# tgialoimtr/cnn_lstm_ctc_ocr

Hardware: AMD Instinct MI355X
Metric: line-crops/sec (train step) at 32x256 bs=256; CER vs ref (higher is better)
Workload: dtype bf16

## Files before the change

### cnn_lstm_ctc_ocr_amd/csrc/gemm.hip

```cpp
#include <atomic>
#include <cstdlib>
#include <type_traits>

#include "gemm.h"
#include "mfma_util.h"

namespace ocrk {

template <int AM, typename CT>
__device__ __forceinline__ const CT* a_addr(const GemmParams& p, const CT* A, int m, int k, bool& ok) {
    if constexpr (AM == A_ROWK) {
        ok = m < p.M && k < p.K;
        return A + (int64_t)m * p.lda + k;
    } else if constexpr (AM == A_COLK) {
        ok = m < p.M && k < p.K;
        return A + (int64_t)k * p.lda + m;
    } else {
        int pix, kidx;
        if constexpr (AM == A_IM2COL_T) { pix = k; kidx = m; ok = k < p.K && m < p.M; }
        else { pix = m; kidx = k; ok = m < p.M && k < p.K; }
        const int C = p.convC, W = p.convW, H = p.convH;
        int tap = kidx / C, c = kidx - tap * C;
        int kh = tap / 3, kw = tap - kh * 3;
        int w = pix % W, t2 = pix / W, h = t2 % H, b = t2 / H;
        int hh, ww;
        if constexpr (AM == A_IM2COL_FLIP) { hh = h - kh + 1; ww = w - kw + 1; }
        else { hh = h + kh - 1; ww = w + kw - 1; }
        ok = ok && hh >= 0 && hh < H && ww >= 0 && ww < W;
        return A + (((int64_t)b * H + hh) * W + ww) * C + c;
    }
}

template <int BMD, typename CT>
__device__ __forceinline__ const CT* b_addr(const GemmParams& p, const CT* B, int n, int k, bool& ok) {
    ok = n < p.N && k < p.K;
    if constexpr (BMD == B_NK) return B + (int64_t)n * p.ldb + k;
    else return B + (int64_t)k * p.ldb + n;
}

template <typename CT, int AM, int BMD, int TBM, int TBN, bool X3 = false>
__global__ void __launch_bounds__(256) gemm_kernel(const GemmParams p) {
    static_assert(!X3 || sizeof(CT) == 4, "bf16x3 splits fp32 operands");
    using RT = typename std::conditional<X3, unsigned short, typename RawT<CT>::T>::type;
    constexpr int BK = 32, LDK = BK + 8;
    constexpr int WM = TBM / 2, WN = TBN / 2, TM = WM / 16, TN = WN / 16;
    constexpr bool A_K = (AM == A_ROWK || AM == A_IM2COL || AM == A_IM2COL_FLIP);
    constexpr bool B_K = (BMD == B_NK);
    constexpr bool BF = sizeof(CT) == 2;
    constexpr bool A_TR = BF && !A_K, B_TR = BF && !B_K;
    constexpr bool PERM = A_TR || B_TR;
    constexpr int LDA_R = TBM + 16, LDB_R = TBN + 16;
    constexpr int A_ELEMS = A_TR ? BK * LDA_R : TBM * LDK;
    constexpr int B_ELEMS = B_TR ? BK * LDB_R : TBN * LDK;
    constexpr int NVA = (TBM * BK / 8 + 255) / 256;
    constexpr int NVB = (TBN * BK / 8 + 255) / 256;
    __shared__ __attribute__((aligned(16))) RT sA[2][X3 ? 2 * A_ELEMS : A_ELEMS];
    __shared__ __attribute__((aligned(16))) RT sB[2][X3 ? 2 * B_ELEMS : B_ELEMS];

    const int tid = threadIdx.x, lane = tid & 63, wave = tid >> 6;
    const int wm = wave >> 1, wn = wave & 1;
    const int m0 = blockIdx.x * TBM, n0 = blockIdx.y * TBN;
    const int zb = blockIdx.z / p.splits, zs = blockIdx.z - zb * p.splits;
    const CT* A = reinterpret_cast<const CT*>(p.A) + zb * p.strideA;
    const CT* B = reinterpret_cast<const CT*>(p.B) + zb * p.strideB;
    const int kbeg = zs * p.k_chunk;
    const int kend = min(p.K, kbeg + p.k_chunk);
    const int nk = max(0, (kend - kbeg + BK - 1) / BK);

    V8<CT> ra[NVA], rb[NVB];
    auto load_tiles = [&](int k0) {
#pragma unroll
        for (int v = 0; v < NVA; ++v) {
            int idx = tid + 256 * v;
            vzero(ra[v]);
            if (idx < TBM * BK / 8) {
                int m, k;
                if constexpr (A_K) { m = m0 + (idx >> 2); k = k0 + 8 * (idx & 3); }
                else { k = k0 + idx / (TBM / 8); m = m0 + 8 * (idx % (TBM / 8)); }
                bool ok;
                const CT* src = a_addr<AM, CT>(p, A, m, k, ok);
                if (ok && k < kend) vload(ra[v], src);
            }
        }
#pragma unroll
        for (int v = 0; v < NVB; ++v) {
            int idx = tid + 256 * v;
            vzero(rb[v]);
            if (idx < TBN * BK / 8) {
                int n, k;
                if constexpr (B_K) { n = n0 + (idx >> 2); k = k0 + 8 * (idx & 3); }
                else { k = k0 + idx / (TBN / 8); n = n0 + 8 * (idx % (TBN / 8)); }
                bool ok;
                const CT* src = b_addr<BMD, CT>(p, B, n, k, ok);
                if (ok && k < kend) vload(rb[v], src);
            }
        }
    };
    auto store_tiles_x3 = [&](int buf) {
        if constexpr (X3) {
#pragma unroll
            for (int v = 0; v < NVA; ++v) {
                int idx = tid + 256 * v;
                if (idx < TBM * BK / 8) {
                    u32x4 hi, lo;
                    split8_bf16(ra[v], hi, lo);
                    if constexpr (A_K) {
                        const int o = (idx >> 2) * LDK + 8 * (idx & 3);
                        *reinterpret_cast<u32x4*>(&sA[buf][o]) = hi;
                        *reinterpret_cast<u32x4*>(&sA[buf][A_ELEMS + o]) = lo;
                    } else {
                        int kk = idx / (TBM / 8), r0 = 8 * (idx % (TBM / 8));
#pragma unroll
                        for (int i = 0; i < 8; ++i) {
                            sA[buf][(r0 + i) * LDK + kk] = (unsigned short)(hi[i >> 1] >> (16 * (i & 1)));
                            sA[buf][A_ELEMS + (r0 + i) * LDK + kk] = (unsigned short)(lo[i >> 1] >> (16 * (i & 1)));
                        }
                    }
                }
            }
#pragma unroll
            for (int v = 0; v < NVB; ++v) {
                int idx = tid + 256 * v;
                if (idx < TBN * BK / 8) {
                    u32x4 hi, lo;
                    split8_bf16(rb[v], hi, lo);
                    if constexpr (B_K) {
                        const int o = (idx >> 2) * LDK + 8 * (idx & 3);
                        *reinterpret_cast<u32x4*>(&sB[buf][o]) = hi;
                        *reinterpret_cast<u32x4*>(&sB[buf][B_ELEMS + o]) = lo;
                    } else {
                        int kk = idx / (TBN / 8), r0 = 8 * (idx % (TBN / 8));
#pragma unroll
                        for (int i = 0; i < 8; ++i) {
                            sB[buf][(r0 + i) * LDK + kk] = (unsigned short)(hi[i >> 1] >> (16 * (i & 1)));
                            sB[buf][B_ELEMS + (r0 + i) * LDK + kk] = (unsigned short)(lo[i >> 1] >> (16 * (i & 1)));
                        }
                    }
                }
            }
        }
    };
    auto store_tiles = [&](int buf) {
        if constexpr (X3) {
            store_tiles_x3(buf);
        } else {
#pragma unroll
        for (int v = 0; v < NVA; ++v) {
            int idx = tid + 256 * v;
            if (idx < TBM * BK / 8) {
                if constexpr (A_K) {
                    vstore_lds(&sA[buf][(idx >> 2) * LDK + 8 * (idx & 3)], ra[v]);
                } else {
                    int kk = idx / (TBM / 8), r0 = 8 * (idx % (TBM / 8));
                    if constexpr (A_TR) {
                        vstore_lds(&sA[buf][kk * LDA_R + r0], ra[v]);
                    } else {
#pragma unroll
                        for (int i = 0; i < 8; ++i) sA[buf][(r0 + i) * LDK + kk] = ra[v].e(i);
                    }
                }
            }
        }
#pragma unroll
        for (int v = 0; v < NVB; ++v) {
            int idx = tid + 256 * v;
            if (idx < TBN * BK / 8) {
                if constexpr (B_K) {
                    vstore_lds(&sB[buf][(idx >> 2) * LDK + 8 * (idx & 3)], rb[v]);
                } else {
                    int kk = idx / (TBN / 8), r0 = 8 * (idx % (TBN / 8));
                    if constexpr (B_TR) {
                        vstore_lds(&sB[buf][kk * LDB_R + r0], rb[v]);
                    } else {
#pragma unroll
                        for (int i = 0; i < 8; ++i) sB[buf][(r0 + i) * LDK + kk] = rb[v].e(i);
                    }
                }
            }
        }
        }
    };

    floatx4 acc[TM][TN];
#pragma unroll
    for (int i = 0; i < TM; ++i)
#pragma unroll
        for (int j = 0; j < TN; ++j) acc[i][j] = floatx4{0.f, 0.f, 0.f, 0.f};

    if (nk > 0) {
        load_tiles(kbeg);
        store_tiles(0);
        __syncthreads();
    }
    const int g = lane >> 4, i16 = lane & 15;
    for (int kt = 0; kt < nk; ++kt) {
        const int buf = kt & 1;
        if (kt + 1 < nk) load_tiles(kbeg + (kt + 1) * BK);
        if constexpr (X3) {
            bf16x8 ah[TM], al[TM], bh[TN], bl[TN];
#pragma unroll
            for (int i = 0; i < TM; ++i) {
                const RT* ap = &sA[buf][(wm * WM + i * 16 + i16) * LDK + 8 * g];
                ah[i] = *reinterpret_cast<const bf16x8*>(ap);
                al[i] = *reinterpret_cast<const bf16x8*>(ap + A_ELEMS);
            }
#pragma unroll
            for (int j = 0; j < TN; ++j) {
                const RT* bp = &sB[buf][(wn * WN + j * 16 + i16) * LDK + 8 * g];
                bh[j] = *reinterpret_cast<const bf16x8*>(bp);
                bl[j] = *reinterpret_cast<const bf16x8*>(bp + B_ELEMS);
            }
#pragma unroll
            for (int i = 0; i < TM; ++i)
#pragma unroll
                for (int j = 0; j < TN; ++j) {
                    acc[i][j] = __builtin_amdgcn_mfma_f32_16x16x32_bf16(al[i], bh[j], acc[i][j], 0, 0, 0);
                    acc[i][j] = __builtin_amdgcn_mfma_f32_16x16x32_bf16(ah[i], bl[j], acc[i][j], 0, 0, 0);
                    acc[i][j] = __builtin_amdgcn_mfma_f32_16x16x32_bf16(ah[i], bh[j], acc[i][j], 0, 0, 0);
                }
        } else if constexpr (BF) {
            bf16x8 af[TM], bfr[TN];
#pragma unroll
            for (int i = 0; i < TM; ++i) {
                if constexpr (A_TR) {
                    const RT* ap = &sA[buf][(4 * g + (i16 >> 2)) * LDA_R + wm * WM + i * 16 + 4 * (i16 & 3)];
                    af[i] = frag_tr(ap, 16 * LDA_R);
                } else {
                    const RT* ap = &sA[buf][(wm * WM + i * 16 + i16) * LDK];
                    af[i] = PERM ? frag_perm(ap, g) : *reinterpret_cast<const bf16x8*>(ap + 8 * g);
                }
            }
#pragma unroll
            for (int j = 0; j < TN; ++j) {
                if constexpr (B_TR) {
                    const RT* bp = &sB[buf][(4 * g + (i16 >> 2)) * LDB_R + wn * WN + j * 16 + 4 * (i16 & 3)];
                    bfr[j] = frag_tr(bp, 16 * LDB_R);
                } else {
                    const RT* bp = &sB[buf][(wn * WN + j * 16 + i16) * LDK];
                    bfr[j] = PERM ? frag_perm(bp, g) : *reinterpret_cast<const bf16x8*>(bp + 8 * g);
                }
            }
#pragma unroll
            for (int i = 0; i < TM; ++i)
#pragma unroll
                for (int j = 0; j < TN; ++j)
                    acc[i][j] = __builtin_amdgcn_mfma_f32_16x16x32_bf16(af[i], bfr[j], acc[i][j], 0, 0, 0);
        } else {
            const RT* a_base = &sA[buf][(wm * WM + i16) * LDK + 8 * g];
            const RT* b_base = &sB[buf][(wn * WN + i16) * LDK + 8 * g];
            V8<float> af[TM], bfr[TN];
#pragma unroll
            for (int i = 0; i < TM; ++i) vload_lds(af[i], a_base + i * 16 * LDK);
#pragma unroll
            for (int j = 0; j < TN; ++j) vload_lds(bfr[j], b_base + j * 16 * LDK);
#pragma unroll
            for (int kk = 0; kk < 8; ++kk)
#pragma unroll
                for (int i = 0; i < TM; ++i)
#pragma unroll
                    for (int j = 0; j < TN; ++j)
                        acc[i][j] = __builtin_amdgcn_mfma_f32_16x16x4f32(af[i].e(kk), bfr[j].e(kk), acc[i][j], 0, 0, 0);
        }
        if (kt + 1 < nk) store_tiles(buf ^ 1);
        __syncthreads();
    }

    const int row_base = m0 + wm * WM + (lane >> 4) * 4;
    const int col_base = n0 + wn * WN + (lane & 15);
    if (p.splits > 1) {
        float* ws = p.splitk_ws + ((int64_t)zb * p.splits + zs) * (int64_t)p.M * p.N;
#pragma unroll
        for (int i = 0; i < TM; ++i)
#pragma unroll
            for (int j = 0; j < TN; ++j)
#pragma unroll
                for (int r = 0; r < 4; ++r) {
                    int row = row_base + i * 16 + r, col = col_base + j * 16;
                    if (row < p.M && col < p.N) ws[(int64_t)row * p.N + col] = acc[i][j][r];
                }
        return;
    }
    const float* bias = p.bias ? p.bias + zb * p.strideBias : nullptr;
    const CT* mask = reinterpret_cast<const CT*>(p.mask);
    float* Cf = reinterpret_cast<float*>(p.C) + zb * p.strideC;
    bf16* Cb = reinterpret_cast<bf16*>(p.C) + zb * p.strideC;
#pragma unroll
    for (int i = 0; i < TM; ++i)
#pragma unroll
        for (int j = 0; j < TN; ++j) {
            int col = col_base + j * 16;
            float bcol = (bias && col < p.N) ? bias[col] : 0.f;
#pragma unroll
            for (int r = 0; r < 4; ++r) {
                int row = row_base + i * 16 + r;
                float v = p.alpha * acc[i][j][r] + bcol;
                if (row < p.M && col < p.N) {
                    if (mask && !(to_f32(mask[(int64_t)row * p.ldmask + col]) > 0.f)) v = 0.f;
                    if (p.relu) v = fmaxf(v, 0.f);
                    int64_t off = (int64_t)row * p.ldc + col;
                    if (p.c_bf16) {
                        Cb[off] = (bf16)v;
                    } else {
                        if (p.accumulate) v += Cf[off];
                        Cf[off] = v;
                    }
                }
                acc[i][j][r] = v;
            }
        }
    if (!p.stats) return;

    __shared__ float s_red[2][TBN];
    const int valid_rows = min(TBM, p.M - m0);
    float tsum[TN];
#pragma unroll
    for (int j = 0; j < TN; ++j) {
        float s = 0.f;
#pragma unroll
        for (int i = 0; i < TM; ++i)
#pragma unroll
            for (int r = 0; r < 4; ++r)
                if (row_base + i * 16 + r < p.M) s += acc[i][j][r];
        s = add_xor32(add_xor16(s));
        tsum[j] = s;
    }
    if (lane < 16)
#pragma unroll
        for (int j = 0; j < TN; ++j) s_red[wm][wn * WN + j * 16 + lane] = tsum[j];
    __syncthreads();
    float tmean[TN];
#pragma unroll
    for (int j = 0; j < TN; ++j) {
        int c = wn * WN + j * 16 + (lane & 15);
        tsum[j] = s_red[0][c] + s_red[1][c];
        tmean[j] = tsum[j] / (float)valid_rows;
    }
    __syncthreads();
#pragma unroll
    for (int j = 0; j < TN; ++j) {
        float s = 0.f;
#pragma unroll
        for (int i = 0; i < TM; ++i)
#pragma unroll
            for (int r = 0; r < 4; ++r)
                if (row_base + i * 16 + r < p.M) {
                    float d = acc[i][j][r] - tmean[j];
                    s += d * d;
                }
        s = add_xor32(add_xor16(s));
        if (lane < 16) s_red[wm][wn * WN + j * 16 + lane] = s;
    }
    __syncthreads();
    if (wm == 0 && lane < 16) {
#pragma unroll
        for (int j = 0; j < TN; ++j) {
            int c = wn * WN + j * 16 + lane;
            if (n0 + c < p.N) {
                float* st = p.stats + (int64_t)blockIdx.x * 2 * p.N;
                st[n0 + c] = tsum[j];
                st[p.N + n0 + c] = s_red[0][c] + s_red[1][c];
            }
        }
    }
}

__global__ void __launch_bounds__(256) splitk_reduce_kernel(const GemmParams p) {
    const int64_t MN = (int64_t)p.M * p.N;
    const int zb = blockIdx.y;
    const float* ws = p.splitk_ws + (int64_t)zb * p.splits * MN;
    const float* bias = p.bias ? p.bias + zb * p.strideBias : nullptr;
    for (int64_t e = (int64_t)blockIdx.x * 256 + threadIdx.x; e < MN; e += (int64_t)gridDim.x * 256) {
        float v = 0.f;
        for (int s = 0; s < p.splits; ++s) v += ws[s * MN + e];
        int row = (int)(e / p.N), col = (int)(e - (int64_t)row * p.N);
        v = p.alpha * v + (bias ? bias[col] : 0.f);
        if (p.relu) v = fmaxf(v, 0.f);
        int64_t off = zb * p.strideC + (int64_t)row * p.ldc + col;
        if (p.c_bf16) {
            reinterpret_cast<bf16*>(p.C)[off] = (bf16)v;
        } else {
            float* C = reinterpret_cast<float*>(p.C);
            C[off] = p.accumulate ? C[off] + v : v;
        }
    }
}

__global__ void __launch_bounds__(256) splitk_reduce4_kernel(const GemmParams p) {
    const int64_t MN = (int64_t)p.M * p.N, n4 = MN / 4;
    const int zb = blockIdx.y;
    const float4* ws = reinterpret_cast<const float4*>(p.splitk_ws + (int64_t)zb * p.splits * MN);
    const float* bias = p.bias ? p.bias + zb * p.strideBias : nullptr;
    for (int64_t e = (int64_t)blockIdx.x * 256 + threadIdx.x; e < n4; e += (int64_t)gridDim.x * 256) {
        float v[4] = {0.f, 0.f, 0.f, 0.f};
        for (int s = 0; s < p.splits; ++s) {
            const float4 u = ws[s * n4 + e];
            v[0] += u.x; v[1] += u.y; v[2] += u.z; v[3] += u.w;
        }
        const int64_t e0 = e * 4;
        const int row = (int)(e0 / p.N), col = (int)(e0 - (int64_t)row * p.N);
#pragma unroll
        for (int j = 0; j < 4; ++j) {
            v[j] = p.alpha * v[j] + (bias ? bias[col + j] : 0.f);
            if (p.relu) v[j] = fmaxf(v[j], 0.f);
        }
        const int64_t off = zb * p.strideC + (int64_t)row * p.ldc + col;
        if (p.c_bf16) {
            union { uint2 q; bf16 h[4]; } o;
#pragma unroll
            for (int j = 0; j < 4; ++j) o.h[j] = (bf16)v[j];
            *reinterpret_cast<uint2*>(reinterpret_cast<bf16*>(p.C) + off) = o.q;
        } else {
            float4* C = reinterpret_cast<float4*>(reinterpret_cast<float*>(p.C) + off);
            float4 c = make_float4(v[0], v[1], v[2], v[3]);
            if (p.accumulate) {
                const float4 o = *C;
                c = make_float4(o.x + v[0], o.y + v[1], o.z + v[2], o.w + v[3]);
            }
            *C = c;
        }
    }
}

__global__ void __launch_bounds__(256) splitk_reduce4p_kernel(const GemmParams p) {
    const int64_t MN = (int64_t)p.M * p.N, n4 = MN / 4;
    const int zb = blockIdx.y;
    const float4* ws = reinterpret_cast<const float4*>(p.splitk_ws + (int64_t)zb * p.splits * MN);
    const int part = threadIdx.x >> 4, ql = threadIdx.x & 15;
    const int64_t e = (int64_t)blockIdx.x * 16 + ql;
    __shared__ float4 red[16][16];
    float4 v = make_float4(0.f, 0.f, 0.f, 0.f);
    if (e < n4) {
        int s = part;
        for (; s + 16 < p.splits; s += 32) {
            const float4 u0 = ws[s * n4 + e], u1 = ws[(s + 16) * n4 + e];
            v.x += u0.x; v.y += u0.y; v.z += u0.z; v.w += u0.w;
            v.x += u1.x; v.y += u1.y; v.z += u1.z; v.w += u1.w;
        }
        if (s < p.splits) {
            const float4 u = ws[s * n4 + e];
            v.x += u.x; v.y += u.y; v.z += u.z; v.w += u.w;
        }
    }
    red[part][ql] = v;
    __syncthreads();
    if (part != 0 || e >= n4) return;
    float r[4] = {0.f, 0.f, 0.f, 0.f};
#pragma unroll
    for (int q = 0; q < 16; ++q) {
        const float4 u = red[q][ql];
        r[0] += u.x; r[1] += u.y; r[2] += u.z; r[3] += u.w;
    }
    const float* bias = p.bias ? p.bias + zb * p.strideBias : nullptr;
    const int64_t e0 = e * 4;
    const int row = (int)(e0 / p.N), col = (int)(e0 - (int64_t)row * p.N);
#pragma unroll
    for (int j = 0; j < 4; ++j) {
        r[j] = p.alpha * r[j] + (bias ? bias[col + j] : 0.f);
        if (p.relu) r[j] = fmaxf(r[j], 0.f);
    }
    const int64_t off = zb * p.strideC + (int64_t)row * p.ldc + col;
    if (p.c_bf16) {
        union { uint2 q; bf16 h[4]; } o;
#pragma unroll
        for (int j = 0; j < 4; ++j) o.h[j] = (bf16)r[j];
        *reinterpret_cast<uint2*>(reinterpret_cast<bf16*>(p.C) + off) = o.q;
    } else {
        float4* C = reinterpret_cast<float4*>(reinterpret_cast<float*>(p.C) + off);
        float4 c = make_float4(r[0], r[1], r[2], r[3]);
        if (p.accumulate) {
            const float4 o = *C;
            c = make_float4(o.x + r[0], o.y + r[1], o.z + r[2], o.w + r[3]);
        }
        *C = c;
    }
}

int splitk_finish(const GemmParams& p, hipStream_t stream) {
    if (p.splits <= 1) return OCRK_OK;
    int64_t MN = (int64_t)p.M * p.N;
    const bool v4 = p.N % 4 == 0 && p.ldc % 4 == 0 && p.strideC % 4 == 0 &&
                    (uintptr_t)p.C % 16 == 0 && (uintptr_t)p.splitk_ws % 16 == 0;
    if (v4 && (p.splits >= 32 || (p.splits >= 8 && MN / 4 < 65536))) {
        dim3 rg((unsigned)cdiv(MN / 4, 16), (unsigned)p.batch);
        splitk_reduce4p_kernel<<<rg, 256, 0, stream>>>(p);
        return launch_status("gemm splitk reduce");
    }
    if (v4) {
        dim3 rg((unsigned)std::min<int64_t>(cdiv(MN / 4, 256), 4096), (unsigned)p.batch);
        splitk_reduce4_kernel<<<rg, 256, 0, stream>>>(p);
        return launch_status("gemm splitk reduce");
    }
    dim3 rg((unsigned)std::min<int64_t>(cdiv(MN, 256), 4096), (unsigned)p.batch);
    splitk_reduce_kernel<<<rg, 256, 0, stream>>>(p);
    return launch_status("gemm splitk reduce");
}

size_t gemm_splitk_ws_bytes(int M, int N, int batch, int splits) {
    return splits > 1 ? (size_t)batch * splits * M * N * sizeof(float) : 0;
}

static std::atomic<int> g_f32_mode{0};

bool f32_exact_mfma() {
    return opt(OPT_F32_MFMA) == 1 || g_f32_mode.load(std::memory_order_relaxed) == 1;
}

template <typename CT, int AM, int BMD>
static int launch_tiles(const GemmParams& p0, hipStream_t stream) {
    GemmParams p = p0;
    int TBM = 128, TBN = p.N <= 32 ? 32 : (p.N <= 64 ? 64 : 128);
    dim3 grid((unsigned)cdiv(p.M, TBM), (unsigned)cdiv(p.N, TBN), (unsigned)(p.batch * p.splits));
    constexpr bool F32 = sizeof(CT) == 4;
    if (F32 && !f32_exact_mfma()) {
        if (TBN == 32) gemm_kernel<CT, AM, BMD, 128, 32, F32><<<grid, 256, 0, stream>>>(p);
        else if (TBN == 64) gemm_kernel<CT, AM, BMD, 128, 64, F32><<<grid, 256, 0, stream>>>(p);
        else gemm_kernel<CT, AM, BMD, 128, 128, F32><<<grid, 256, 0, stream>>>(p);
    } else if (TBN == 32) gemm_kernel<CT, AM, BMD, 128, 32><<<grid, 256, 0, stream>>>(p);
    else if (TBN == 64) gemm_kernel<CT, AM, BMD, 128, 64><<<grid, 256, 0, stream>>>(p);
    else gemm_kernel<CT, AM, BMD, 128, 128><<<grid, 256, 0, stream>>>(p);
    int st = launch_status("gemm");
    if (st != OCRK_OK) return st;
    return splitk_finish(p, stream);
}

template <typename CT>
static int dispatch_modes(const GemmParams& p, int amode, int bmode, hipStream_t s) {
#define GM(AMx, BMx) if (amode == AMx && bmode == BMx) return launch_tiles<CT, AMx, BMx>(p, s)
    GM(A_ROWK, B_NK);
    GM(A_ROWK, B_KN);
    GM(A_COLK, B_KN);
    GM(A_IM2COL, B_NK);
    GM(A_IM2COL_FLIP, B_NK);
    GM(A_IM2COL_T, B_KN);
#undef GM
    set_error("gemm: unsupported operand modes A=%d B=%d", amode, bmode);
    return OCRK_ERR_INVALID_ARG;
}

int gemm(const GemmParams& p, int amode, int bmode, int dtype, hipStream_t stream) {
    if (p.M <= 0 || p.N <= 0 || p.batch <= 0) return OCRK_OK;
    OCRK_REQUIRE(p.K >= 0 && p.splits >= 1 && p.k_chunk > 0 && p.k_chunk % 32 == 0,
                 "gemm: bad K=%d splits=%d k_chunk=%d", p.K, p.splits, p.k_chunk);
    bool a_rows = (amode == A_COLK || amode == A_IM2COL_T);
    OCRK_REQUIRE(p.K % 8 == 0 || (a_rows && bmode == B_KN),
                 "gemm: K=%d must be a multiple of 8 for k-contiguous operands", p.K);
    OCRK_REQUIRE(!a_rows || p.M % 8 == 0, "gemm: M=%d must be a multiple of 8 for this A mode", p.M);
    OCRK_REQUIRE(bmode != B_KN || p.N % 8 == 0, "gemm: N=%d must be a multiple of 8 for B_KN", p.N);
    OCRK_REQUIRE(amode < A_IM2COL || p.convC % 8 == 0, "gemm: conv channels must be a multiple of 8");
    OCRK_REQUIRE(!(p.stats && (p.splits > 1 || p.batch > 1)), "gemm: stats need splits=1, batch=1");
    OCRK_REQUIRE(!(p.accumulate && p.c_bf16), "gemm: accumulate needs an f32 C");
    if (p.mask_bits || p.relu_bits) {
        const int st = gemm_nt(p, amode, bmode, dtype, stream);
        OCRK_REQUIRE(st >= 0, "gemm: ReLU bit masks need the NT engine (bf16 C, staged epilogue) for this shape");
        return st;
    }
    int nt = gemm_w4(p, amode, bmode, dtype, stream);
    if (nt < 0) nt = gemm_pp(p, amode, bmode, dtype, stream);
    if (nt >= 0) return nt != OCRK_OK ? nt : splitk_finish(p, stream);
    nt = gemm_nt(p, amode, bmode, dtype, stream);
    if (nt < 0) nt = gemm_w4tn(p, amode, bmode, dtype, stream);
    if (nt < 0) nt = gemm_pptn(p, amode, bmode, dtype, stream);
    if (nt < 0) nt = gemm_tn(p, amode, bmode, dtype, stream);
    if (nt >= 0) return nt != OCRK_OK ? nt : splitk_finish(p, stream);
    if (dtype == OCRK_BF16) return dispatch_modes<bf16>(p, amode, bmode, stream);
    if (dtype == OCRK_F32) return dispatch_modes<float>(p, amode, bmode, stream);
    set_error("gemm: unsupported dtype %d", dtype);
    return OCRK_ERR_INVALID_ARG;
}

}

extern "C" int ocrk_set_f32_gemm_mode(int mode) {
    OCRK_REQUIRE(mode == 0 || mode == 1, "ocrk_set_f32_gemm_mode: mode %d not 0 (bf16x3) or 1 (exact)", mode);
    return ocrk::g_f32_mode.exchange(mode);
}

extern "C" int ocrk_f32_gemm_exact(void) { return ocrk::f32_exact_mfma() ? 1 : 0; }

extern "C" size_t ocrk_gemm_workspace_size(int M, int N, int batch, int splits) {
    return ocrk::gemm_splitk_ws_bytes(M, N, batch, splits);
}

extern "C" int ocrk_gemm(int trans_a, int trans_b, int M, int N, int K, float alpha, const void* A,
                         int64_t lda, int64_t stride_a, const void* B, int64_t ldb, int64_t stride_b,
                         void* C, int64_t ldc, int64_t stride_c, int c_dtype, const float* bias,
                         int relu, int accumulate, int batch, int dtype, int splits, void* ws,
                         size_t ws_bytes, void* stream) {
    ocrk::GemmParams p = {};
    p.M = M; p.N = N; p.K = K; p.batch = batch < 1 ? 1 : batch;
    p.A = A; p.lda = lda; p.strideA = stride_a;
    p.B = B; p.ldb = ldb; p.strideB = stride_b;
    p.C = C; p.ldc = ldc; p.strideC = stride_c;
    p.c_bf16 = c_dtype == OCRK_BF16;
    p.bias = bias; p.strideBias = 0;
    p.relu = relu; p.accumulate = accumulate; p.alpha = alpha;
    p.splits = splits < 1 ? 1 : splits;
    int kc = (int)ocrk::cdiv(K, p.splits);
    p.k_chunk = (int)ocrk::cdiv(kc < 32 ? 32 : kc, 32) * 32;
    p.splits = (int)ocrk::cdiv(K > 0 ? K : 1, p.k_chunk);
    p.splitk_ws = (float*)ws;
    OCRK_REQUIRE(p.splits == 1 || ws_bytes >= ocrk::gemm_splitk_ws_bytes(M, N, p.batch, p.splits),
                 "ocrk_gemm: split-K workspace too small");
    int amode = trans_a ? ocrk::A_COLK : ocrk::A_ROWK;
    int bmode = trans_b ? ocrk::B_NK : ocrk::B_KN;
    return ocrk::gemm(p, amode, bmode, dtype, ocrk::as_stream(stream));
}
```

### cnn_lstm_ctc_ocr_amd/csrc/gemm_w4.hip

```cpp
#include "gemm.h"
#include "mfma_util.h"

namespace ocrk {

namespace {

constexpr unsigned W4_OOB = 0x80000000u;

__device__ __forceinline__ void w4_barrier() {
    __builtin_amdgcn_sched_barrier(0);
    asm volatile("" ::: "memory");
    __builtin_amdgcn_s_barrier();
    asm volatile("" ::: "memory");
    __builtin_amdgcn_sched_barrier(0);
}

template <int NR, int NM, int REST>
__device__ __forceinline__ void w4_interleave() {
#pragma unroll
    for (int r = 0; r < NR; ++r) {
        __builtin_amdgcn_sched_group_barrier(0x8, NM, 0);
        __builtin_amdgcn_sched_group_barrier(0x100, 1, 0);
    }
    __builtin_amdgcn_sched_group_barrier(0x8, REST, 0);
}

typedef unsigned short u16x4 __attribute__((ext_vector_type(4)));

__device__ __forceinline__ i32x4_t w4_rsrc(const void* base, int bytes) {
    const uint64_t b = (uint64_t)base;
    return i32x4_t{(int)(unsigned)b, (int)((unsigned)(b >> 32) & 0xffffu), bytes, 0x00020000};
}

__device__ __forceinline__ void w4_dma16(const i32x4_t& r, unsigned lds, unsigned voff, unsigned soff) {
    asm volatile("s_nop 0\n\tbuffer_load_dwordx4 %0, %1, %2 offen lds"
                 :: "v"(voff), "s"(r), "s"(soff), "{m0}"(lds) : "memory");
}

template <int BN>
__global__ void __launch_bounds__(256) gemm_w4_kernel(const GemmParams p) {
    constexpr int BM = 256, BK = 64, ROWB = 128;
    constexpr int WN = BN / 2, NJ = WN / 16;
    constexpr int A_BYTES = BM * ROWB, BUF = (BM + BN) * ROWB;
    constexpr int NU = 8, NUB = BN / 32;
    constexpr int NB = 2;
    constexpr int BIAS_OFF = NB * BUF, STG_OFF = BIAS_OFF + 4 * 1024;
    constexpr int PITCH = WN * 2 + 16, STG = 16 * PITCH;
    constexpr int CL = WN / 8, RPS = 64 / CL;
    constexpr int NST = 8 * (16 / RPS);
    extern __shared__ __attribute__((aligned(16))) char smem[];

    const int tid = threadIdx.x, lane = tid & 63;
    const int wave = __builtin_amdgcn_readfirstlane(tid >> 6);
    const int wm = wave >> 1, wn = wave & 1;
    const int i16 = lane & 15, g = lane >> 4, sw = lane & 7;

    const int tm = (p.M + BM - 1) / BM, tn = (p.N + BN - 1) / BN;
    const int nitems = tm * tn * p.batch;
    const int per = (nitems + 7) >> 3;
    const int xcd = blockIdx.x & 7, slot = blockIdx.x >> 3, sp = gridDim.x >> 3;
    const int wend = min(nitems, (xcd + 1) * per);
    int w_issue = xcd * per + slot;
    if (w_issue >= wend) return;

    typedef const __attribute__((address_space(4))) GemmParams* KArgs;
    const bool has_bias = p.bias != nullptr;
    const int c_nk = max(1, (p.K + BK - 1) / BK);

    const int lrow = lane >> 3;
    const int cs = (lane & 7) ^ lrow;
    i32x4_t ra, rb;
    int i_m0 = 0, i_n0 = 0, i_zb = 0, i_kt = 0, i_cnt = 0;
    const unsigned a_lane = (unsigned)(lrow * p.lda * 2), b_lane = (unsigned)(lrow * p.ldb * 2);
    auto setup_issue = [&](int w) {
        const PPItem it = pp_item(w, tm, tn, 1, BM, BN);
        ra = w4_rsrc(reinterpret_cast<const bf16*>(p.A) + it.zb * p.strideA, p.M * (int)p.lda * 2);
        rb = w4_rsrc(reinterpret_cast<const bf16*>(p.B) + it.zb * p.strideB, p.N * (int)p.ldb * 2);
        i_m0 = it.m0;
        i_n0 = it.n0;
        i_zb = it.zb;
        i_kt = 0;
    };
    int ops = 0;
    const unsigned lds0 = (unsigned)(uintptr_t)(__attribute__((address_space(3))) char*)smem;
    auto lane_off = [&](unsigned lane_row, bool on) -> unsigned {
        const int k = i_kt * BK + 8 * cs;
        return on && k < p.K ? lane_row + (unsigned)(k * 2) : W4_OOB;
    };
    auto unit_base = [&](int first, unsigned buf, int& row, unsigned& lds) {
        row = first + wave * 8;
        lds = buf + wave * 8 * ROWB;
        asm volatile("" : "+s"(row), "+s"(lds));
    };
    auto dma_a = [&](int i, int row, unsigned lds, unsigned va) {
        const int mrow = row + i * 32;
        const unsigned soff = mrow < p.M ? (unsigned)(mrow * (int)p.lda * 2) : 0u;
        w4_dma16(ra, lds + i * 32 * ROWB, lrow < p.M - mrow ? va : W4_OOB, soff);
    };
    auto dma_b = [&](int i, int row, unsigned lds, unsigned vb) {
        const int ncol = row + i * 32;
        const unsigned soff = ncol < p.N ? (unsigned)(ncol * (int)p.ldb * 2) : 0u;
        w4_dma16(rb, lds + i * 32 * ROWB, lrow < p.N - ncol ? vb : W4_OOB, soff);
    };
    auto dma_bias = [&](bool on) {
        if (i_kt == 0 && has_bias && wave == 0) {
            const int n = i_n0 + 4 * lane;
            KArgs e = (KArgs)__builtin_amdgcn_kernarg_segment_ptr();
            asm volatile("" : "+s"(e));
            const i32x4_t rbias = w4_rsrc(e->bias + i_zb * e->strideBias, p.N * 4);
            w4_dma16(rbias, lds0 + BIAS_OFF + (i_cnt & 3) * 1024, on && 4 * lane < BN && n < p.N ? (unsigned)(n * 4) : W4_OOB, 0u);
            ops += 1;
        }
    };
    auto advance_issue = [&]() -> bool {
        if (++i_kt < c_nk) return true;
        w_issue += sp;
        ++i_cnt;
        if (w_issue >= wend) return false;
        setup_issue(w_issue);
        return true;
    };

    int w_comp = w_issue, c_cnt = 0;

    bf16x8 af0[8], bf0[NJ], af1[8], bf1[NJ];
    const int a_base = (wm * 128 + i16) * ROWB, b_base = A_BYTES + (wn * WN + i16) * ROWB;
    auto read_a = [&](const char* buf, int kk, bf16x8 (&fr)[8]) {
#pragma unroll
        for (int i = 0; i < 8; ++i)
            fr[i] = *reinterpret_cast<const bf16x8*>(buf + a_base + i * 16 * ROWB + (((kk * 4 + g) ^ sw) << 4));
    };
    auto read_b = [&](const char* buf, int kk, bf16x8 (&fr)[NJ]) {
#pragma unroll
        for (int j = 0; j < NJ; ++j)
            fr[j] = *reinterpret_cast<const bf16x8*>(buf + b_base + j * 16 * ROWB + (((kk * 4 + g) ^ sw) << 4));
    };
    floatx4 acc[8][NJ];
    (void)read_b;

    int mA[NB + 1] = {}, mB[NB + 1] = {};
    setup_issue(w_issue);
    bool more = true;
#pragma unroll
    for (int t = 0; t < NB; ++t) {
        const unsigned va = lane_off(a_lane, more), vb = lane_off(b_lane, more);
        int row;
        unsigned lds;
        unit_base(i_m0, lds0 + t * BUF, row, lds);
#pragma unroll
        for (int i = 0; i < NU; ++i) dma_a(i, row, lds, va);
        ops += NU;
        mA[t] = ops;
        dma_bias(more);
        unit_base(i_n0, lds0 + t * BUF + A_BYTES, row, lds);
#pragma unroll
        for (int i = 0; i < NUB; ++i) dma_b(i, row, lds, vb);
        ops += NUB;
        mB[t] = ops;
        if (more) more = advance_issue();
    }
    vm_wait_n(ops - mB[0]);
    w4_barrier();
    read_a(smem, 0, af0);
    read_b(smem, 0, bf0);

    int s = 0;
    auto k_tile = [&](auto FIRST_) {
        constexpr bool FIRST = decltype(FIRST_)::value;
        char* cur = smem + (s & 1) * BUF;
        const char* nxt = smem + ((s + 1) & 1) * BUF;
        __builtin_amdgcn_sched_barrier(0);
        __builtin_amdgcn_s_setprio(1);
        read_a(cur, 1, af1);
        read_b(cur, 1, bf1);
#pragma unroll
        for (int i = 0; i < 8; ++i)
#pragma unroll
            for (int j = 0; j < NJ; ++j) {
                if constexpr (FIRST)
                    acc[i][j] = __builtin_amdgcn_mfma_f32_16x16x32_bf16(bf0[j], af0[i], floatx4{0.f, 0.f, 0.f, 0.f}, 0, 0, 0);
                else acc[i][j] = __builtin_amdgcn_mfma_f32_16x16x32_bf16(bf0[j], af0[i], acc[i][j], 0, 0, 0);
            }
        if constexpr (NJ == 8) w4_interleave<16, 3, 16>();
        else w4_interleave<12, 2, 8>();
        __builtin_amdgcn_s_setprio(0);
        __builtin_amdgcn_sched_barrier(0);
        asm volatile("s_waitcnt lgkmcnt(0)" ::: "memory");
        vm_wait_fast<NUB>(ops - mA[1]);
        w4_barrier();
        {
            const unsigned va = lane_off(a_lane, more);
            int row;
            unsigned lds;
            unit_base(i_m0, lds0 + (s & 1) * BUF, row, lds);
            __builtin_amdgcn_s_setprio(1);
#pragma unroll
            for (int q = 0; q < 8; ++q) {
                af0[q] = *reinterpret_cast<const bf16x8*>(nxt + a_base + q * 16 * ROWB + ((g ^ sw) << 4));
#pragma unroll
                for (int t = q * (NJ / 2); t < (q + 1) * (NJ / 2); ++t)
                    acc[t / NJ][t % NJ] =
                        __builtin_amdgcn_mfma_f32_16x16x32_bf16(bf1[t % NJ], af1[t / NJ], acc[t / NJ][t % NJ], 0, 0, 0);
                dma_a(q, row, lds, va);
                __builtin_amdgcn_sched_barrier(0);
            }
            __builtin_amdgcn_s_setprio(0);
            ops += NU;
            mA[NB] = ops;
        }
        vm_wait_fast<NU>(ops - mB[1]);
        w4_barrier();
        {
            const unsigned vb = lane_off(b_lane, more);
            dma_bias(more);
            int row;
            unsigned lds;
            unit_base(i_n0, lds0 + (s & 1) * BUF + A_BYTES, row, lds);
            __builtin_amdgcn_s_setprio(1);
#pragma unroll
            for (int q = 0; q < NJ; ++q) {
                bf0[q] = *reinterpret_cast<const bf16x8*>(nxt + b_base + q * 16 * ROWB + ((g ^ sw) << 4));
#pragma unroll
                for (int t = q * 4; t < q * 4 + 4; ++t)
                    acc[4 + t / NJ][t % NJ] = __builtin_amdgcn_mfma_f32_16x16x32_bf16(bf1[t % NJ], af1[4 + t / NJ],
                                                                                      acc[4 + t / NJ][t % NJ], 0, 0, 0);
                dma_b(q, row, lds, vb);
                __builtin_amdgcn_sched_barrier(0);
            }
            __builtin_amdgcn_s_setprio(0);
            ops += NUB;
            mB[NB] = ops;
        }
        if (more) more = advance_issue();
        mA[1] = mA[2];
        mB[1] = mB[2];
        ++s;
    };

    for (;;) {
        k_tile(std::true_type{});
        for (int c_kt = 1; c_kt < c_nk; ++c_kt) k_tile(std::false_type{});

        {
            int el;
            asm volatile("v_mbcnt_lo_u32_b32 %0, -1, 0\n\tv_mbcnt_hi_u32_b32 %0, -1, %0" : "=v"(el));
            const PPItem cur_it = pp_item(w_comp, tm, tn, 1, BM, BN);
            KArgs e = (KArgs)__builtin_amdgcn_kernarg_segment_ptr();
            asm volatile("" : "+s"(e));
            const int i16 = el & 15, g = el >> 4;
            const char* bslot = smem + BIAS_OFF + (c_cnt & 3) * 1024 + (wn * WN + 4 * g) * 4;
            floatx4 bv[NJ];
#pragma unroll
            for (int j = 0; j < NJ; ++j) {
                bv[j] = floatx4{0.f, 0.f, 0.f, 0.f};
                if (has_bias) bv[j] = *reinterpret_cast<const floatx4*>(bslot + j * 64);
            }
            char* stg = smem + STG_OFF + wave * STG;
            bf16* Cb = reinterpret_cast<bf16*>(e->C) + cur_it.zb * e->strideC;
            const __amdgpu_buffer_rsrc_t rc =
                __builtin_amdgcn_make_buffer_rsrc(Cb, 0, ((p.M - 1) * (int)e->ldc + p.N) * 2, 0x00020000);
            const int c8 = el & (CL - 1), r0 = el / CL;
            const int n = cur_it.n0 + wn * WN + 8 * c8;
#pragma unroll
            for (int h = 0; h < 8; ++h) {
#pragma unroll
                for (int j = 0; j < NJ; ++j) {
                    floatx4 v = acc[h][j] * e->alpha + bv[j];
                    if (e->relu) {
#pragma unroll
                        for (int r = 0; r < 4; ++r) v[r] = fmaxf(v[r], 0.f);
                    }
                    u16x4 o;
#pragma unroll
                    for (int r = 0; r < 4; ++r) o[r] = __builtin_bit_cast(unsigned short, (bf16)v[r]);
                    *reinterpret_cast<u16x4*>(stg + i16 * PITCH + (j * 16 + 4 * g) * 2) = o;
                }
                __builtin_amdgcn_wave_barrier();
#pragma unroll
                for (int q = 0; q < 16 / RPS; ++q) {
                    const int r = r0 + q * RPS;
                    const int m = cur_it.m0 + wm * 128 + h * 16 + r;
                    const u32x4 v = *reinterpret_cast<const u32x4*>(stg + r * PITCH + c8 * 16);
                    const unsigned off = (m < p.M && n < p.N) ? (unsigned)(((int64_t)m * e->ldc + n) * 2) : W4_OOB;
                    __builtin_amdgcn_raw_buffer_store_b128(v, rc, off, 0, 0);
                }
                __builtin_amdgcn_wave_barrier();
            }
            ops += NST;
        }
        w_comp += sp;
        ++c_cnt;
        if (w_comp >= wend) break;
    }
    vm_wait<0>();
}

}

int gemm_w4(const GemmParams& p, int amode, int bmode, int dtype, hipStream_t stream) {
    const int64_t mode = opt(OPT_GEMM_W4);
    if (mode == 0 || dtype != OCRK_BF16 || amode != A_ROWK || bmode != B_NK) return -1;
    if (!p.c_bf16 || p.accumulate || p.splits != 1 || p.mask || p.stats || p.mask_bits || p.relu_bits) return -1;
    if (p.N % 8 != 0 || p.K % 8 != 0 || (int64_t)p.M < 4096 || p.N < 96) return -1;
    if ((int64_t)p.M * p.lda * 2 >= (1ll << 31) || (int64_t)p.N * p.ldb * 2 >= (1ll << 31) ||
        (int64_t)p.M * p.ldc * 2 >= (1ll << 31))
        return -1;
    if (p.ldc % 8 != 0 || p.strideC % 8 != 0 || (uintptr_t)p.C % 16 != 0) return -1;
    if (p.bias && (uintptr_t)p.bias % 16 != 0) return -1;
    if (p.lda % 8 != 0 || p.ldb % 8 != 0) return -1;
    if (mode == 1 && (p.K < 1024 || p.N < 256)) return -1;
    const int ncu = cu_count();
    const bool narrow = 2 * cdiv(p.M, 256) * cdiv(p.N, 256) * (int64_t)p.batch <= ncu;
    const int bn = narrow ? 128 : 256;
    const int lds = 2 * (256 + bn) * 128 + 4 * 1024 + 4 * 16 * (bn + 16);
    static DeviceOnce configured[2];
    const void* kern = narrow ? reinterpret_cast<const void*>(&gemm_w4_kernel<128>)
                              : reinterpret_cast<const void*>(&gemm_w4_kernel<256>);
    set_dyn_lds(configured[narrow ? 1 : 0], kern, lds);
    const int64_t items = cdiv(p.M, 256) * cdiv(p.N, bn) * (int64_t)p.batch;
    const int64_t grid = std::min<int64_t>(cdiv(items, 8) * 8, (int64_t)(ncu / 8) * 8);
    if (narrow) gemm_w4_kernel<128><<<dim3((unsigned)grid), 256, lds, stream>>>(p);
    else gemm_w4_kernel<256><<<dim3((unsigned)grid), 256, lds, stream>>>(p);
    opt_add(OPT_GEMM_W4_LAUNCHES, 1);
    return launch_status("gemm_w4");
}

}
```

Baseline: 55910.

## Run implicit-GEMM 3x3 convolutions on the w4 DMA-to-LDS GEMM engine

Adds conv (im2col and flipped im2col) modes to the w4 persistent GEMM kernel. A rows are gathered directly from the NHWC activation through buffer-load-to-LDS with per-row tap masks for padding, and an optional fused ReLU bit-mask output is written from the epilogue. Conv GEMMs and ReLU-bit GEMMs previously went through the NT/PP engines. The w4 path is also tried first in the dispatcher. The added mask and index arithmetic and the extra bit-mask stores add work, and the fixed 256x128 tile may fit some conv shapes poorly.

```diff
diff --git a/cnn_lstm_ctc_ocr_amd/csrc/gemm.hip b/cnn_lstm_ctc_ocr_amd/csrc/gemm.hip
--- a/cnn_lstm_ctc_ocr_amd/csrc/gemm.hip
+++ b/cnn_lstm_ctc_ocr_amd/csrc/gemm.hip
@@ -549,13 +549,14 @@
     OCRK_REQUIRE(amode < A_IM2COL || p.convC % 8 == 0, "gemm: conv channels must be a multiple of 8");
     OCRK_REQUIRE(!(p.stats && (p.splits > 1 || p.batch > 1)), "gemm: stats need splits=1, batch=1");
     OCRK_REQUIRE(!(p.accumulate && p.c_bf16), "gemm: accumulate needs an f32 C");
+    int nt = gemm_w4(p, amode, bmode, dtype, stream);
+    if (nt >= 0) return nt;
     if (p.mask_bits || p.relu_bits) {
         const int st = gemm_nt(p, amode, bmode, dtype, stream);
         OCRK_REQUIRE(st >= 0, "gemm: ReLU bit masks need the NT engine (bf16 C, staged epilogue) for this shape");
         return st;
     }
-    int nt = gemm_w4(p, amode, bmode, dtype, stream);
-    if (nt < 0) nt = gemm_pp(p, amode, bmode, dtype, stream);
+    nt = gemm_pp(p, amode, bmode, dtype, stream);
     if (nt >= 0) return nt != OCRK_OK ? nt : splitk_finish(p, stream);
     nt = gemm_nt(p, amode, bmode, dtype, stream);
     if (nt < 0) nt = gemm_w4tn(p, amode, bmode, dtype, stream);
diff --git a/cnn_lstm_ctc_ocr_amd/csrc/gemm_w4.hip b/cnn_lstm_ctc_ocr_amd/csrc/gemm_w4.hip
--- a/cnn_lstm_ctc_ocr_amd/csrc/gemm_w4.hip
+++ b/cnn_lstm_ctc_ocr_amd/csrc/gemm_w4.hip
@@ -37,9 +37,11 @@
                  :: "v"(voff), "s"(r), "s"(soff), "{m0}"(lds) : "memory");
 }
 
-template <int BN>
+template <int BN, int CONV = 0>
 __global__ void __launch_bounds__(256) gemm_w4_kernel(const GemmParams p) {
     constexpr int BM = 256, BK = 64, ROWB = 128;
+    constexpr bool IM = CONV != 0, FLIP = CONV == 2;
+    static_assert(!IM || BN == 128, "the conv forms run on the 256 x 128 tile");
     constexpr int WN = BN / 2, NJ = WN / 16;
     constexpr int A_BYTES = BM * ROWB, BUF = (BM + BN) * ROWB;
     constexpr int NU = 8, NUB = BN / 32;
@@ -71,10 +73,47 @@
     const int cs = (lane & 7) ^ lrow;
     i32x4_t ra, rb;
     int i_m0 = 0, i_n0 = 0, i_zb = 0, i_kt = 0, i_cnt = 0;
-    const unsigned a_lane = (unsigned)(lrow * p.lda * 2), b_lane = (unsigned)(lrow * p.ldb * 2);
+    const unsigned a_lane = IM ? (unsigned)((lrow * p.convC + 8 * cs) * 2) : (unsigned)(lrow * p.lda * 2);
+    const unsigned b_lane = (unsigned)(lrow * p.ldb * 2);
+    unsigned tmask[IM ? 8 : 1];
+    int i_tap = 0, i_cc = 0;
+    const int d32w = IM ? 32 % p.convW : 0, d32h = IM ? (32 / p.convW) % p.convH : 0;
+    const float rcpw = IM ? 1.f / (float)p.convW : 0.f, rcph = IM ? 1.f / (float)p.convH : 0.f;
+    auto setup_masks = [&](int m0) {
+        if constexpr (IM) {
+            const int W = p.convW, H = p.convH;
+            asm volatile("" : "+s"(m0));
+            const int m = m0 + wave * 8 + lrow;
+            int q = (int)((float)m * rcpw), w = m - q * W;
+            if (w < 0) { w += W; --q; }
+            if (w >= W) { w -= W; ++q; }
+            int q2 = (int)((float)q * rcph), h = q - q2 * H;
+            if (h < 0) h += H;
+            if (h >= H) h -= H;
+#pragma unroll
+            for (int i = 0; i < 8; ++i) {
+                const unsigned wm = (w > 0 ? 1u : 0u) | 2u | (w < W - 1 ? 4u : 0u);
+                unsigned mk = wm << 3;
+                if (h > 0) mk |= wm;
+                if (h < H - 1) mk |= wm << 6;
+                tmask[i] = m + 32 * i < p.M ? mk : 0u;
+                w += d32w;
+                h += d32h;
+                if (w >= W) { w -= W; ++h; }
+                if (h >= H) h -= H;
+            }
+        }
+    };
     auto setup_issue = [&](int w) {
         const PPItem it = pp_item(w, tm, tn, 1, BM, BN);
-        ra = w4_rsrc(reinterpret_cast<const bf16*>(p.A) + it.zb * p.strideA, p.M * (int)p.lda * 2);
+        if constexpr (IM) {
+            ra = w4_rsrc(p.A, p.M * p.convC * 2);
+            setup_masks(it.m0);
+            i_tap = 0;
+            i_cc = 0;
+        } else {
+            ra = w4_rsrc(reinterpret_cast<const bf16*>(p.A) + it.zb * p.strideA, p.M * (int)p.lda * 2);
+        }
         rb = w4_rsrc(reinterpret_cast<const bf16*>(p.B) + it.zb * p.strideB, p.N * (int)p.ldb * 2);
         i_m0 = it.m0;
         i_n0 = it.n0;
@@ -92,8 +131,23 @@
         lds = buf + wave * 8 * ROWB;
         asm volatile("" : "+s"(row), "+s"(lds));
     };
+    unsigned abit = 0;
+    auto lane_off_a = [&](bool on) -> unsigned {
+        if constexpr (IM) {
+            const int kh = (i_tap * 11) >> 5, kw = i_tap - 3 * kh;
+            const int sh = (kh - 1) * p.convW + kw - 1;
+            abit = on ? 1u << (FLIP ? 8 - i_tap : i_tap) : 0u;
+            return a_lane + (unsigned)(((FLIP ? -sh : sh) * p.convC + i_cc) * 2);
+        } else {
+            return lane_off(a_lane, on);
+        }
+    };
     auto dma_a = [&](int i, int row, unsigned lds, unsigned va) {
         const int mrow = row + i * 32;
+        if constexpr (IM) {
+            w4_dma16(ra, lds + i * 32 * ROWB, (tmask[i] & abit) ? va + (unsigned)(mrow * p.convC * 2) : W4_OOB, 0u);
+            return;
+        }
         const unsigned soff = mrow < p.M ? (unsigned)(mrow * (int)p.lda * 2) : 0u;
         w4_dma16(ra, lds + i * 32 * ROWB, lrow < p.M - mrow ? va : W4_OOB, soff);
     };
@@ -113,7 +167,16 @@
         }
     };
     auto advance_issue = [&]() -> bool {
-        if (++i_kt < c_nk) return true;
+        if (++i_kt < c_nk) {
+            if constexpr (IM) {
+                i_cc += BK;
+                if (i_cc >= p.convC) {
+                    i_cc = 0;
+                    ++i_tap;
+                }
+            }
+            return true;
+        }
         w_issue += sp;
         ++i_cnt;
         if (w_issue >= wend) return false;
@@ -143,7 +206,7 @@
     bool more = true;
 #pragma unroll
     for (int t = 0; t < NB; ++t) {
-        const unsigned va = lane_off(a_lane, more), vb = lane_off(b_lane, more);
+        const unsigned va = lane_off_a(more), vb = lane_off(b_lane, more);
         int row;
         unsigned lds;
         unit_base(i_m0, lds0 + t * BUF, row, lds);
@@ -189,7 +252,7 @@
         vm_wait_fast<NUB>(ops - mA[1]);
         w4_barrier();
         {
-            const unsigned va = lane_off(a_lane, more);
+            const unsigned va = lane_off_a(more);
             int row;
             unsigned lds;
             unit_base(i_m0, lds0 + (s & 1) * BUF, row, lds);
@@ -261,6 +324,12 @@
                 __builtin_amdgcn_make_buffer_rsrc(Cb, 0, ((p.M - 1) * (int)e->ldc + p.N) * 2, 0x00020000);
             const int c8 = el & (CL - 1), r0 = el / CL;
             const int n = cur_it.n0 + wn * WN + 8 * c8;
+            bool bits = false;
+            __amdgpu_buffer_rsrc_t rbits = rc;
+            if constexpr (IM) {
+                bits = e->relu_bits != nullptr;
+                rbits = __builtin_amdgcn_make_buffer_rsrc(e->relu_bits, 0, p.M * (p.N >> 3), 0x00020000);
+            }
 #pragma unroll
             for (int h = 0; h < 8; ++h) {
 #pragma unroll
@@ -283,10 +352,26 @@
                     const u32x4 v = *reinterpret_cast<const u32x4*>(stg + r * PITCH + c8 * 16);
                     const unsigned off = (m < p.M && n < p.N) ? (unsigned)(((int64_t)m * e->ldc + n) * 2) : W4_OOB;
                     __builtin_amdgcn_raw_buffer_store_b128(v, rc, off, 0, 0);
+                    if constexpr (IM) {
+                        if (bits) {
+                            unsigned mb = 0;
+#pragma unroll
+                            for (int t = 0; t < 4; ++t) {
+                                mb |= (__uint_as_float(v[t] << 16) > 0.f ? 1u : 0u) << (2 * t);
+                                mb |= (__uint_as_float(v[t] & 0xffff0000u) > 0.f ? 1u : 0u) << (2 * t + 1);
+                            }
+                            unsigned x = mb << (8 * (el & 3));
+                            x |= (unsigned)__builtin_amdgcn_update_dpp(0, (int)x, 0xB1, 0xf, 0xf, true);
+                            x |= (unsigned)__builtin_amdgcn_update_dpp(0, (int)x, 0x4E, 0xf, 0xf, true);
+                            const unsigned boff = ((el & 3) == 0 && m < p.M && n < p.N)
+                                                      ? (unsigned)(m * (p.N >> 3) + (n >> 3)) : W4_OOB;
+                            __builtin_amdgcn_raw_buffer_store_b32(x, rbits, boff, 0, 0);
+                        }
+                    }
                 }
                 __builtin_amdgcn_wave_barrier();
             }
-            ops += NST;
+            ops += bits ? 2 * NST : NST;
         }
         w_comp += sp;
         ++c_cnt;
@@ -299,8 +384,15 @@
 
 int gemm_w4(const GemmParams& p, int amode, int bmode, int dtype, hipStream_t stream) {
     const int64_t mode = opt(OPT_GEMM_W4);
-    if (mode == 0 || dtype != OCRK_BF16 || amode != A_ROWK || bmode != B_NK) return -1;
-    if (!p.c_bf16 || p.accumulate || p.splits != 1 || p.mask || p.stats || p.mask_bits || p.relu_bits) return -1;
+    const bool conv = amode == A_IM2COL || amode == A_IM2COL_FLIP;
+    if (mode == 0 || dtype != OCRK_BF16 || (amode != A_ROWK && !conv) || bmode != B_NK) return -1;
+    if (!p.c_bf16 || p.accumulate || p.splits != 1 || p.mask || p.stats || p.mask_bits) return -1;
+    if (p.relu_bits && !conv) return -1;
+    if (conv) {
+        if (p.batch != 1 || p.convC % 64 != 0 || p.K != 9 * p.convC || p.convH < 1 || p.convW < 1) return -1;
+        if ((int64_t)p.M >= (1ll << 24) || (int64_t)p.M * p.convC * 2 >= (1ll << 31)) return -1;
+        if (p.relu_bits && (p.N % 32 != 0 || p.ldc != p.N || (uintptr_t)p.relu_bits % 4 != 0)) return -1;
+    }
     if (p.N % 8 != 0 || p.K % 8 != 0 || (int64_t)p.M < 4096 || p.N < 96) return -1;
     if ((int64_t)p.M * p.lda * 2 >= (1ll << 31) || (int64_t)p.N * p.ldb * 2 >= (1ll << 31) ||
         (int64_t)p.M * p.ldc * 2 >= (1ll << 31))
@@ -308,18 +400,24 @@
     if (p.ldc % 8 != 0 || p.strideC % 8 != 0 || (uintptr_t)p.C % 16 != 0) return -1;
     if (p.bias && (uintptr_t)p.bias % 16 != 0) return -1;
     if (p.lda % 8 != 0 || p.ldb % 8 != 0) return -1;
-    if (mode == 1 && (p.K < 1024 || p.N < 256)) return -1;
+    if (mode == 1 && !conv && (p.K < 1024 || p.N < 256)) return -1;
+    if (mode == 1 && conv) return -1;
     const int ncu = cu_count();
-    const bool narrow = 2 * cdiv(p.M, 256) * cdiv(p.N, 256) * (int64_t)p.batch <= ncu;
+    const bool narrow = conv || 2 * cdiv(p.M, 256) * cdiv(p.N, 256) * (int64_t)p.batch <= ncu;
     const int bn = narrow ? 128 : 256;
     const int lds = 2 * (256 + bn) * 128 + 4 * 1024 + 4 * 16 * (bn + 16);
-    static DeviceOnce configured[2];
-    const void* kern = narrow ? reinterpret_cast<const void*>(&gemm_w4_kernel<128>)
-                              : reinterpret_cast<const void*>(&gemm_w4_kernel<256>);
-    set_dyn_lds(configured[narrow ? 1 : 0], kern, lds);
+    static DeviceOnce configured[4];
+    const int ki = amode == A_IM2COL ? 2 : amode == A_IM2COL_FLIP ? 3 : narrow ? 1 : 0;
+    const void* kern = ki == 2   ? reinterpret_cast<const void*>(&gemm_w4_kernel<128, 1>)
+                       : ki == 3 ? reinterpret_cast<const void*>(&gemm_w4_kernel<128, 2>)
+                       : ki == 1 ? reinterpret_cast<const void*>(&gemm_w4_kernel<128>)
+                                 : reinterpret_cast<const void*>(&gemm_w4_kernel<256>);
+    set_dyn_lds(configured[ki], kern, lds);
     const int64_t items = cdiv(p.M, 256) * cdiv(p.N, bn) * (int64_t)p.batch;
     const int64_t grid = std::min<int64_t>(cdiv(items, 8) * 8, (int64_t)(ncu / 8) * 8);
-    if (narrow) gemm_w4_kernel<128><<<dim3((unsigned)grid), 256, lds, stream>>>(p);
+    if (ki == 2) gemm_w4_kernel<128, 1><<<dim3((unsigned)grid), 256, lds, stream>>>(p);
+    else if (ki == 3) gemm_w4_kernel<128, 2><<<dim3((unsigned)grid), 256, lds, stream>>>(p);
+    else if (narrow) gemm_w4_kernel<128><<<dim3((unsigned)grid), 256, lds, stream>>>(p);
     else gemm_w4_kernel<256><<<dim3((unsigned)grid), 256, lds, stream>>>(p);
     opt_add(OPT_GEMM_W4_LAUNCHES, 1);
     return launch_status("gemm_w4");
```

Result: no change. 55950 (median of 5 runs) (+0.1%).
